# drapado/PINGS

Measured on AMD Instinct MI355X. Metric: raster fwd+bwd Mpix/s @1M Gaussians 1080p, higher is better.
Workload: dtype f32; 1 GPU; surfel rasteriser fwd+bwd, 1000000 Gaussians, 1920x1080, one view per GPU; gaussians=1000000, width=1920, height=1080

## Files before the change

### pings_amd/csrc/raster_blend_fwd.hip

```cpp
#include "raster_common.hpp"

namespace pings {
namespace raster {

template <int MODE>
__device__ __forceinline__ void blend_fwd_wave_body(
    const KParams& p, const uint2* __restrict__ ranges, const uint32_t* __restrict__ point_list,
    const float4* __restrict__ rec, const uint32_t* __restrict__ gval, float* __restrict__ out_color,
    float* __restrict__ out_normal, float* __restrict__ out_depth, float* __restrict__ out_alpha,
    float* __restrict__ final_T, uint32_t* __restrict__ n_contrib, float* __restrict__ inst_wq,
    uint32_t* __restrict__ inst_cntq, const uint32_t* __restrict__ tile_order,
    const uint32_t* __restrict__ seg_tile_unit0, const unsigned block) {
  __shared__ float4 sA_[4][64], sB_[4][64], sC_[4][64], sD_[4][64];
  __shared__ uint32_t sSlot_[4][64];
  __shared__ int sE_[4][64];
  __shared__ float sW_[4][64];
  __shared__ uint32_t sCnt_[4][64];

  const int lane = threadIdx.x & 63, q = (int)(threadIdx.x >> 6);
  float4 *sA = sA_[q], *sB = sB_[q], *sC = sC_[q], *sD = sD_[q];
  uint32_t *sSlot = sSlot_[q], *sCnt = sCnt_[q];
  int* sE = sE_[q];
  float* sW = sW_[q];
  const int tile = (int)tile_order[block];
// ... 714 lines not shown
  for (int k = 0; k < PPL; ++k) {
    if (!inside[k]) continue;
    const int r = k >> 1, h = k & 1;
    const float Tk = T[r][h];
    const size_t pix_id = (size_t)pix_y[r] * p.W + pix_x[h];
    const float A = 1.0f - Tk;
    final_T[pix_id] = Tk;
    n_contrib[pix_id] = last[k];
    out_color[pix_id] = C0[r][h] + Tk * p.bg[0];
    out_color[HW + pix_id] = C1[r][h] + Tk * p.bg[1];
    out_color[2 * HW + pix_id] = C2[r][h] + Tk * p.bg[2];
    out_alpha[pix_id] = A;
    if (MODE == MODE_SURFEL) {
      out_normal[pix_id] = N0[r][h];
      out_normal[HW + pix_id] = N1[r][h];
      out_normal[2 * HW + pix_id] = N2[r][h];
      out_depth[pix_id] = D[r][h] / fmaxf(A, DEPTH_ALPHA_EPS);
    } else {
      out_depth[pix_id] = D[r][h];
    }
  }
  uint32_t mc = 0u;
#pragma unroll
  for (int k = 0; k < PPL; ++k) mc = max(mc, inside[k] ? last[k] : 0u);
#pragma unroll
  for (int off = 32; off > 0; off >>= 1) mc = max(mc, (uint32_t)__shfl_xor((int)mc, off, 64));
  if (lane == 0) tile_maxc[tile] = mc;
}

template <int MODE>
__global__ __launch_bounds__(256) void combine_quadrants_kernel(int64_t I, const float4* __restrict__ wq,
                                                                const uint4* __restrict__ cq, float* __restrict__ inst_w,
                                                                uint32_t* __restrict__ inst_cnt,
                                                                uint8_t* __restrict__ inst_qmask) {
  const int64_t i = (int64_t)blockIdx.x * blockDim.x + threadIdx.x;
  if (i == 0) { inst_w[I] = 0.f; inst_qmask[I] = 0; }
  if (i >= I) return;
  const float4 w = wq[i];
  inst_w[i] = ((w.x + w.y) + w.z) + w.w;
  inst_qmask[i] = (uint8_t)((w.x != 0.f ? 1u : 0u) | (w.y != 0.f ? 2u : 0u) | (w.z != 0.f ? 4u : 0u) | (w.w != 0.f ? 8u : 0u));
  if (MODE == MODE_3DGS) {
    const uint4 c = cq[i];
    inst_cnt[i] = c.x + c.y + c.z + c.w;
  }
}

__device__ inline uint32_t wave_reduce_sum_u32(uint32_t v) {
#pragma unroll
  for (int off = 32; off > 0; off >>= 1) v += (uint32_t)__shfl_xor((int)v, off, 64);
  return v;
}

constexpr int SMALL_RUN = 16;
template <typename T>
__global__ __launch_bounds__(256) void per_gaussian_sum_kernel(
    int P, const uint4* __restrict__ rect, const uint32_t* __restrict__ rank_of,
    const uint32_t* __restrict__ offsets_sorted, const uint32_t* __restrict__ tiles_sorted,
    const T* __restrict__ inst, T* __restrict__ out) {
  const int g = blockIdx.x * blockDim.x + threadIdx.x;
  const int lane = threadIdx.x & 63;
  uint32_t n = 0, base = 0;
  if (g < P && rect[g].w != 0u) {
    const uint32_t r = rank_of[g];
    n = tiles_sorted[r];
    base = offsets_sorted[r] - n;
  }
  T sum = (T)0;
  if (n <= (uint32_t)SMALL_RUN)
    for (uint32_t k = 0; k < n; ++k) sum += inst[base + k];
  unsigned long long m = __ballot(n > (uint32_t)SMALL_RUN);
  while (m) {
    const int src = __ffsll((long long)m) - 1;
    m &= m - 1;
    const uint32_t nb = lane_value(n, src);
    const uint32_t bb = lane_value(base, src);
    T acc = (T)0, acc1 = (T)0, acc2 = (T)0, acc3 = (T)0;
    uint32_t k = lane;
    for (; k + 192 < nb; k += 256) {
      acc += inst[bb + k];
      acc1 += inst[bb + k + 64];
      acc2 += inst[bb + k + 128];
      acc3 += inst[bb + k + 192];
    }
    for (; k < nb; k += 64) acc += inst[bb + k];
    acc = (acc + acc1) + (acc2 + acc3);
    if constexpr (sizeof(T) == 4 && !std::is_integral<T>::value) {
      acc = wave_sum_to_all(acc);
    } else {
      acc = (T)wave_reduce_sum_u32((uint32_t)acc);
    }
    if (lane == src) sum = acc;
  }
  if (g < P) out[g] = sum;
}

struct FwdOut {
  float *color, *normal, *depth, *alpha;
};

template <int MODE>
static int launch_blend_fwd_wave(const KParams& kp, const BlendPlan& plan, int64_t I, int num_tiles, const GeomState& gs,
                          const BinState& bs, const ImageState& im, const FwdOut& o, hipStream_t st) {
  const uint32_t seg = plan.seg;
  if (I > 0) PINGS_HIP_CHECK(hipMemsetAsync(bs.inst_wq, 0, 16 * (size_t)I, st));
  if (I > 0 && MODE == MODE_3DGS) PINGS_HIP_CHECK(hipMemsetAsync(bs.inst_cntq, 0, 16 * (size_t)I, st));
  if (!plan.seg_on) {
    hipLaunchKernelGGL((blend_fwd_wave_kernel<MODE>), dim3(num_tiles), dim3(256), 0, st, kp, bs.ranges,
                       bs.point_list, gs.rec, bs.gval, o.color, o.normal, o.depth, o.alpha,
                       im.final_T, im.n_contrib, bs.inst_wq, bs.inst_cntq, bs.tile_order,
                       (const uint32_t*)nullptr);
  } else {
    hipLaunchKernelGGL(seg_plan_kernel, dim3(1), dim3(1024), 0, st, bs.ranges, num_tiles, 2u * seg, seg,
                       bs.seg_max_units, bs.seg_head, bs.seg_unit_tile, bs.seg_unit_seg, bs.seg_tile_unit0);
    PINGS_LAUNCH_CHECK();
    const dim3 gseg(bs.seg_max_units);
    uint16_t* const rel = plan.seg_reuse ? bs.seg_rel : nullptr;
    uint32_t* const nrel = plan.seg_reuse ? bs.seg_nrel : nullptr;
    hipLaunchKernelGGL((blend_fwd_wave_segT_kernel<MODE>), dim3((unsigned)num_tiles + bs.seg_max_units), dim3(256), 0,
                       st, kp, bs.ranges, bs.point_list, gs.rec, bs.gval, o.color, o.normal, o.depth,
                       o.alpha, im.final_T, im.n_contrib, bs.inst_wq, bs.inst_cntq, bs.tile_order,
                       bs.seg_tile_unit0, (unsigned)num_tiles, seg, bs.seg_head, bs.seg_unit_tile,
                       bs.seg_unit_seg, bs.seg_P, rel, nrel);
    if (plan.seg_reuse)
      hipLaunchKernelGGL((blend_fwd_seg_kernel<MODE, 1, true>), gseg, dim3(256), 0, st, kp, bs.ranges, bs.point_list,
                         gs.rec, bs.gval, seg, bs.seg_head, bs.seg_unit_tile, bs.seg_unit_seg, bs.seg_P, bs.seg_slab,
                         bs.inst_wq, bs.inst_cntq, rel, nrel);
    else
      hipLaunchKernelGGL((blend_fwd_seg_kernel<MODE, 1, false>), gseg, dim3(256), 0, st, kp, bs.ranges, bs.point_list,
                         gs.rec, bs.gval, seg, bs.seg_head, bs.seg_unit_tile, bs.seg_unit_seg, bs.seg_P, bs.seg_slab,
                         bs.inst_wq, bs.inst_cntq, rel, nrel);
    hipLaunchKernelGGL((blend_fwd_seg_combine_kernel<MODE>), gseg, dim3(256), 0, st, kp, bs.ranges, seg, bs.seg_head,
                       bs.seg_unit_tile, bs.seg_unit_seg, bs.seg_slab, o.color, o.normal, o.depth,
                       o.alpha, im.final_T, im.n_contrib);
    PINGS_LAUNCH_CHECK();
  }
  if (I > 0)
    hipLaunchKernelGGL((combine_quadrants_kernel<MODE>), dim3((unsigned)pings::ceil_div<int64_t>(I, 256)),
                       dim3(256), 0, st, I, reinterpret_cast<const float4*>(bs.inst_wq),
                       reinterpret_cast<const uint4*>(bs.inst_cntq), bs.inst_w, bs.inst_cnt, bs.inst_qmask);
  PINGS_LAUNCH_CHECK();
  return PINGS_OK;
}

int launch_blend_fwd(int mode, const KParams& kp, const BlendPlan& plan, int P, int64_t I, const GeomState& gs,
                     const BinState& bs, const ImageState& im, float* out_color, float* out_normal, float* out_depth,
                     float* out_alpha, void* per_gaussian, hipStream_t st) {
  const int num_tiles = kp.gx * kp.gy;
  const FwdOut o{out_color, out_normal, out_depth, out_alpha};
  {
    pings::prof::Scope ps_blend("blend_fwd", st);
    const int e = with_mode(mode, [&](auto m) -> int {
      constexpr int M = m();
      switch (plan.fwd) {
        case BlendPlan::FWD_TILE:
          hipLaunchKernelGGL((blend_fwd_tile_kernel<M>), dim3(num_tiles), dim3(64), 0, st, kp, bs.ranges,
                             bs.point_list, gs.rec, bs.gval, o.color, o.normal, o.depth, o.alpha,
                             im.final_T, im.n_contrib, bs.inst_w, bs.inst_cnt, bs.tile_order, bs.tile_maxc);
          break;
        case BlendPlan::FWD_WAVE:
          if (int e = launch_blend_fwd_wave<M>(kp, plan, I, num_tiles, gs, bs, im, o, st)) return e;
      }
      PINGS_LAUNCH_CHECK();
      return PINGS_OK;
    });
    if (e) return e;
  }
  if (P > 0) {
    pings::prof::Scope ps("per_gaussian_sum", st);
    const dim3 grid(pings::ceil_div(P, 256)), block(256);
    if (I == 0) {
      PINGS_HIP_CHECK(hipMemsetAsync(per_gaussian, 0, 4 * (size_t)P, st));
    } else if (mode == PINGS_RASTER_SURFEL) {
      hipLaunchKernelGGL(per_gaussian_sum_kernel<float>, grid, block, 0, st, P, gs.rect, gs.rank_of,
                         gs.offsets_sorted, gs.tiles_sorted, (const float*)bs.inst_w,
                         reinterpret_cast<float*>(per_gaussian));
    } else {
      hipLaunchKernelGGL(per_gaussian_sum_kernel<uint32_t>, grid, block, 0, st, P, gs.rect, gs.rank_of,
                         gs.offsets_sorted, gs.tiles_sorted, (const uint32_t*)bs.inst_cnt,
                         reinterpret_cast<uint32_t*>(per_gaussian));
    }
    PINGS_LAUNCH_CHECK();
  }
  return PINGS_OK;
}

}
}
```

### pings_amd/csrc/raster_bwd.hip

```cpp
#include <hipcub/hipcub.hpp>

#include <algorithm>
#include <type_traits>

#include "raster_common.hpp"

namespace pings {
namespace raster {

constexpr int BATCH = 64;
constexpr uint32_t LONG_TILES_MAX = 2048;
constexpr uint32_t DEAD_ROW = 0xFFFFFFFFu;

template <int MODE>
__device__ __forceinline__ void blend_bwd_tile_body(
    BParams p, const uint2* __restrict__ ranges, const uint32_t* __restrict__ point_list,
    const float4* __restrict__ rec, const uint32_t* __restrict__ gval, const float* __restrict__ final_T,
    const uint32_t* __restrict__ n_contrib, const float* __restrict__ out_depth, const float* __restrict__ dL_dcolor,
    const float* __restrict__ dL_dnormal, const float* __restrict__ dL_ddepth, const float* __restrict__ dL_dalpha,
    const float* __restrict__ inst_w, const uint32_t* __restrict__ cidx, float* __restrict__ rows,
    const uint32_t* __restrict__ tile_order) {
  __shared__ float4 sA[BATCH], sB[BATCH], sC[BATCH], sD[BATCH];
  __shared__ uint32_t sRow[BATCH];
  __shared__ float4 sG[BATCH][4];
// ... 567 lines not shown
        dst[2] = make_float4(v[8], v[9], v[10], v[11]);
        dst[3] = make_float4(v[12], v[13], v[14], v[15]);
      }
    } else {
      if (gl == lane) {
#pragma unroll
        for (int k = 0; k < 16; ++k) sV[wv][k][lane] = v[k];
      }
      __syncthreads();
      if (act && gl == lane) {
        float o4[4];
#pragma unroll
        for (int u = 0; u < 4; ++u) {
          const int k = 4 * wv + u;
          o4[u] = ((sV[0][k][lane] + sV[1][k][lane]) + sV[2][k][lane]) + sV[3][k][lane];
        }
        dst[wv] = make_float4(o4[0], o4[1], o4[2], o4[3]);
      }
      __syncthreads();
    }
  }
#ifdef PINGS_BWD_STATS
  if (lane == 0) {
    atomicAdd(&g_bwd_stats[0], st_chunks); atomicAdd(&g_bwd_stats[1], st_dead); atomicAdd(&g_bwd_stats[2], st_any);
    atomicAdd(&g_bwd_stats[3], st_exec); atomicAdd(&g_bwd_stats[4], st_valid); atomicAdd(&g_bwd_stats[5], st_take);
  }
#endif
}


__global__ __launch_bounds__(256) void row_chunk_sum_kernel(RowRanges rr, const uint32_t* __restrict__ pair_off,
                                                             const uint32_t* __restrict__ pair_owner,
                                                             const float* __restrict__ rows,
                                                             float* __restrict__ partials) {
  const uint32_t q = (uint32_t)((blockIdx.x * (size_t)blockDim.x + threadIdx.x) >> 4);
  const int c = threadIdx.x & 15;
  if (q >= pair_off[rr.P]) return;
  const uint32_t r = pair_owner[q];
  const uint32_t j = q - pair_off[r];
  const uint32_t row_end = rr.row_end(r);
  uint32_t row = rr.row_begin(r) + j * (uint32_t)CH;
  const uint32_t stop = min(row + (uint32_t)CH, row_end);
  float a0 = 0.f, a1 = 0.f, a2 = 0.f, a3 = 0.f;
  for (; row + 4 <= stop; row += 4) {
    a0 += rows[(size_t)row * 16 + c];
    a1 += rows[(size_t)(row + 1) * 16 + c];
    a2 += rows[(size_t)(row + 2) * 16 + c];
    a3 += rows[(size_t)(row + 3) * 16 + c];
  }
  for (; row < stop; ++row) a0 += rows[(size_t)row * 16 + c];
  partials[(size_t)q * 16 + c] = (a0 + a1) + (a2 + a3);
}

template <int MODE>
__global__ __launch_bounds__(256, 4) void gaussian_bwd_kernel(
    BParams p, const float* __restrict__ means3D, const float* __restrict__ scales,
    const float* __restrict__ rotations, const uint4* __restrict__ rect, const uint32_t* __restrict__ rank_of,
    const uint32_t* __restrict__ tiles_sorted, const uint32_t* __restrict__ pair_off,
    const float* __restrict__ partials, float* __restrict__ dL_dmeans3D, float* __restrict__ dL_dmeans2D, float* __restrict__ dL_dcolors,
    float* __restrict__ dL_dopacities, float* __restrict__ dL_dscales,
    float* __restrict__ dL_drotations, float* __restrict__ tau_partials) {
  __shared__ float sTau[256 / 64][6];
  const int g = blockIdx.x * blockDim.x + threadIdx.x;
  float tau[6] = {0.f, 0.f, 0.f, 0.f, 0.f, 0.f};

  if (g < p.P) {
    uint32_t n_tiles = 0u, qa = 0u, qb = 0u;
    if (rect[g].w != 0u) {
      const uint32_t rank = rank_of[g];
      n_tiles = tiles_sorted[rank];
      qa = pair_off[rank];
      qb = pair_off[rank + 1];
    }
    float G[16];
#pragma unroll
    for (int k = 0; k < 16; ++k) G[k] = 0.f;
    const float4* prow = reinterpret_cast<const float4*>(partials);
    for (uint32_t k = qa; k < qb; ++k) {
#pragma unroll
      for (int q4 = 0; q4 < 4; ++q4) {
        const float4 r = prow[(size_t)k * 4 + q4];
        G[q4 * 4 + 0] += r.x;
        G[q4 * 4 + 1] += r.y;
        G[q4 * 4 + 2] += r.z;
        G[q4 * 4 + 3] += r.w;
      }
    }

    float gm[3] = {0.f, 0.f, 0.f}, gs[3] = {0.f, 0.f, 0.f}, gq4[4] = {0.f, 0.f, 0.f, 0.f};
    float g2d[2] = {0.f, 0.f};
    if (n_tiles > 0 && qb > qa) {
      const float* V = p.view;
      const float* Pm = p.proj_raw;
      const float x = means3D[3 * g], y = means3D[3 * g + 1], z = means3D[3 * g + 2];
      const float px = ((V[0] * x + V[4] * y) + V[8] * z) + V[12];
      const float py = ((V[1] * x + V[5] * y) + V[9] * z) + V[13];
      const float pz = ((V[2] * x + V[6] * y) + V[10] * z) + V[14];
      float gp[3] = {0.f, 0.f, 0.f};
      {
        const float hx = ((Pm[0] * px + Pm[4] * py) + Pm[8] * pz) + Pm[12];
        const float hy = ((Pm[1] * px + Pm[5] * py) + Pm[9] * pz) + Pm[13];
        const float hw = ((Pm[3] * px + Pm[7] * py) + Pm[11] * pz) + Pm[15];
        const float pw = 1.0f / (hw + 1e-7f);
        const float gndx = 0.5f * (float)p.W * G[G_MX];
        const float gndy = 0.5f * (float)p.H * G[G_MY];
        g2d[0] = gndx;
// ... 99 lines not shown
          for (int a = 0; a < 3; ++a) gWc[a][b] += sgn * gn[a] * R[b][2];
        }
        gpz_direct += G[G_ZLO] + G[G_ZHI];
        const float grz = 3.0f * (G[G_ZHI] - G[G_ZLO]);
        if (S[0] > S[1]) gS[0] += grz;
        else if (S[1] > S[0]) gS[1] += grz;
        else { gS[0] += 0.5f * grz; gS[1] += 0.5f * grz; }
      }
      gp[2] += gpz_direct;
      gq4[0] = 2.0f * (-qz * gR[0][1] + qy * gR[0][2] + qz * gR[1][0] - qx * gR[1][2] - qy * gR[2][0] + qx * gR[2][1]);
      gq4[1] = 2.0f * (qy * gR[0][1] + qz * gR[0][2] + qy * gR[1][0] - 2.0f * qx * gR[1][1] - qr * gR[1][2] + qz * gR[2][0] + qr * gR[2][1] - 2.0f * qx * gR[2][2]);
      gq4[2] = 2.0f * (-2.0f * qy * gR[0][0] + qx * gR[0][1] + qr * gR[0][2] + qx * gR[1][0] + qz * gR[1][2] - qr * gR[2][0] + qz * gR[2][1] - 2.0f * qy * gR[2][2]);
      gq4[3] = 2.0f * (-2.0f * qz * gR[0][0] - qr * gR[0][1] + qx * gR[0][2] + qr * gR[1][0] - 2.0f * qz * gR[1][1] + qy * gR[1][2] + qx * gR[2][0] + qy * gR[2][1]);
#pragma unroll
      for (int k = 0; k < 3; ++k) gs[k] = p.scale_mod * gS[k];
#pragma unroll
      for (int b = 0; b < 3; ++b)
        gm[b] = (V[4 * b + 0] * gp[0] + V[4 * b + 1] * gp[1]) + V[4 * b + 2] * gp[2];
      tau[0] = gp[0]; tau[1] = gp[1]; tau[2] = gp[2];
      float th0 = py * gp[2] - pz * gp[1];
      float th1 = pz * gp[0] - px * gp[2];
      float th2 = px * gp[1] - py * gp[0];
#pragma unroll
      for (int b = 0; b < 3; ++b) {
        const float w0 = V[4 * b + 0], w1 = V[4 * b + 1], w2 = V[4 * b + 2];
        th0 += w1 * gWc[2][b] - w2 * gWc[1][b];
        th1 += w2 * gWc[0][b] - w0 * gWc[2][b];
        th2 += w0 * gWc[1][b] - w1 * gWc[0][b];
      }
      tau[3] = th0; tau[4] = th1; tau[5] = th2;
    }
    dL_dmeans3D[3 * g] = gm[0]; dL_dmeans3D[3 * g + 1] = gm[1]; dL_dmeans3D[3 * g + 2] = gm[2];
    dL_dmeans2D[3 * g] = g2d[0]; dL_dmeans2D[3 * g + 1] = g2d[1]; dL_dmeans2D[3 * g + 2] = 0.f;
    dL_dcolors[3 * g] = G[G_R]; dL_dcolors[3 * g + 1] = G[G_G]; dL_dcolors[3 * g + 2] = G[G_B];
    dL_dopacities[g] = G[G_OPAC];
    dL_dscales[3 * g] = gs[0]; dL_dscales[3 * g + 1] = gs[1]; dL_dscales[3 * g + 2] = gs[2];
    dL_drotations[4 * g] = gq4[0]; dL_drotations[4 * g + 1] = gq4[1];
    dL_drotations[4 * g + 2] = gq4[2]; dL_drotations[4 * g + 3] = gq4[3];
  }

  const int lane = threadIdx.x & 63, wave = threadIdx.x >> 6;
#pragma unroll
  for (int k = 0; k < 6; ++k) {
    const float s = wave_reduce_sum_dpp(tau[k]);
    if (lane == 63) sTau[wave][k] = s;
  }
  __syncthreads();
  if (threadIdx.x < 6) {
    const int k = threadIdx.x;
    tau_partials[(size_t)blockIdx.x * 6 + k] = ((sTau[0][k] + sTau[1][k]) + sTau[2][k]) + sTau[3][k];
  }
}

__global__ __launch_bounds__(256) void tau_reduce_kernel(const float* __restrict__ partials, int nblocks,
                                                          float* __restrict__ dL_dtau) {
  __shared__ double sRed[4][6];
  double s[6] = {0, 0, 0, 0, 0, 0};
  for (int i = threadIdx.x; i < nblocks; i += 256) {
#pragma unroll
    for (int k = 0; k < 6; ++k) s[k] += (double)partials[(size_t)i * 6 + k];
  }
#pragma unroll
  for (int k = 0; k < 6; ++k) {
#pragma unroll
    for (int off = 32; off > 0; off >>= 1) s[k] += __shfl_down(s[k], off, 64);
    if ((threadIdx.x & 63) == 0) sRed[threadIdx.x >> 6][k] = s[k];
  }
  __syncthreads();
  if (threadIdx.x < 6)
    dL_dtau[threadIdx.x] = (float)(((sRed[0][threadIdx.x] + sRed[1][threadIdx.x]) + sRed[2][threadIdx.x]) + sRed[3][threadIdx.x]);
}

}
}

using namespace pings::raster;

PINGS_API int pings_raster_backward(const pings_raster_settings* s, int P, int64_t I,
                                    const float* means3D, const float* colors,
                                    const float* opacities, const float* scales,
                                    const float* rotations, const void* geom_blob,
                                    const void* binning_blob, const void* image_blob,
                                    const float* out_color, const float* out_normal,
                                    const float* out_depth, const float* out_alpha,
                                    const float* dL_dcolor, const float* dL_dnormal,
                                    const float* dL_ddepth, const float* dL_dalpha,
                                    void* bwd_blob, float* dL_dmeans3D, float* dL_dmeans2D,
                                    float* dL_dcolors, float* dL_dopacities, float* dL_dscales,
                                    float* dL_drotations, float* dL_dtau, int footprint_class,
                                    void* stream) {
  BParams bp;
  if (int e = fill_camera(s, P, bp)) return e;
  PINGS_ARG_CHECK(dL_dtau != nullptr, "null dL_dtau");
  hipStream_t st = pings::as_stream(stream);
  if (P == 0) {
    PINGS_HIP_CHECK(hipMemsetAsync(dL_dtau, 0, 6 * sizeof(float), st));
    return PINGS_OK;
  }
  PINGS_ARG_CHECK(P > 0 && means3D && colors && opacities && scales && rotations && geom_blob &&
                      binning_blob && image_blob && out_depth && bwd_blob && dL_dmeans3D &&
                      dL_dmeans2D && dL_dcolors && dL_dopacities && dL_dscales && dL_drotations,
                  "null pointer");
  PINGS_ARG_CHECK(I >= 0 && I < (int64_t)0x7FFFFFF0, "instance count out of range");
  (void)out_color; (void)out_normal; (void)out_alpha;
  const RasterKnobs knobs = read_knobs();
  const int num_tiles = bp.gx * bp.gy;
// ... 15 lines not shown
      PINGS_LAUNCH_CHECK();
    }
    order_job.work = fwd_left_it ? bs.tile_maxc : bs.tile_work;
    order_job.num_tiles = num_tiles;
    order_job.order = bs.tile_order + num_tiles;
    order_job.n_long = bs.tile_order + 2 * (size_t)num_tiles;
    order_job.long_thr = plan.long_thr;
    order_job.long_max = LONG_TILES_MAX;
  }
  {
    pings::prof::Scope ps("live_scan", st);
    if (I > 0 && plan.bwd_scan) {
      if (int e = raster_scan_pop(bs.inst_qmask, I + 1, bw.cidx, bw.temp, bw.temp_bytes, knobs.library_scan, order_job, st))
        return e;
    } else if (I > 0) {
      if (int e = raster_scan_live(bs.inst_w, I + 1, bw.cidx, bw.temp, bw.temp_bytes, knobs.library_scan, order_job, st))
        return e;
    } else {
      PINGS_HIP_CHECK(hipMemsetAsync(bw.cidx, 0, 2 * sizeof(uint32_t), st));
    }
    if (int e = raster_scan_chunks(rr, bw.pair_off, bw.pair_owner, bw.temp, bw.temp_bytes, knobs.library_scan, st))
      return e;
  }
  if (I > 0) {
    pings::prof::Scope ps("blend_bwd", st);
    const uint32_t* order = bs.tile_order + num_tiles;
    with_mode(s->mode, [&](auto m) {
      constexpr int M = m();
      if (plan.bwd_scan) {
        const uint32_t* n_long = bs.tile_order + 2 * (size_t)num_tiles;
        const unsigned grid_s = (unsigned)(num_tiles + 3 * std::min<long long>(num_tiles, LONG_TILES_MAX));
        hipLaunchKernelGGL((blend_bwd_scan_kernel<M>), dim3(grid_s), dim3(256), 0, st, bp, bs.ranges,
                           bs.point_list, gs.rec, bs.gval, im.final_T, im.n_contrib, out_depth, dL_dcolor, dL_dnormal,
                           dL_ddepth, dL_dalpha, bs.inst_qmask, bw.cidx, bw.rows, order, n_long);
      } else {
        hipLaunchKernelGGL((blend_bwd_tile_kernel<M>), dim3(num_tiles), dim3(64), 0, st, bp, bs.ranges,
                           bs.point_list, gs.rec, bs.gval, im.final_T, im.n_contrib, out_depth, dL_dcolor,
                           dL_dnormal, dL_ddepth, dL_dalpha, bs.inst_w, bw.cidx, bw.rows, order);
      }
    });
    PINGS_LAUNCH_CHECK();
  }
  {
    pings::prof::Scope ps("row_chunk_sum", st);
    const size_t groups = bw.np_max;
    hipLaunchKernelGGL(row_chunk_sum_kernel, dim3((unsigned)pings::ceil_div<size_t>(groups * 16, 256)),
                       block, 0, st, rr, bw.pair_off, bw.pair_owner, bw.rows, bw.partials);
    PINGS_LAUNCH_CHECK();
  }
  const int nblocks = pings::ceil_div(P, 256);
  {
    pings::prof::Scope ps_g("gaussian_bwd", st);
    with_mode(s->mode, [&](auto m) {
      hipLaunchKernelGGL(gaussian_bwd_kernel<m()>, dim3(nblocks), block, 0, st, bp, means3D,
                         scales, rotations, gs.rect, gs.rank_of, gs.tiles_sorted, bw.pair_off, bw.partials,
                         dL_dmeans3D, dL_dmeans2D, dL_dcolors, dL_dopacities, dL_dscales,
                         dL_drotations, bw.tau_partials);
    });
    PINGS_LAUNCH_CHECK();
    hipLaunchKernelGGL(tau_reduce_kernel, dim3(1), block, 0, st, bw.tau_partials, nblocks, dL_dtau);
    PINGS_LAUNCH_CHECK();
  }
  return PINGS_OK;
}

#ifdef PINGS_BWD_STATS
PINGS_API int pings_debug_bwd_stats(unsigned long long* out8, int reset) {
  PINGS_HIP_CHECK(hipDeviceSynchronize());
  PINGS_HIP_CHECK(hipMemcpyFromSymbol(out8, HIP_SYMBOL(pings::raster::g_bwd_stats), 64));
  if (reset) {
    unsigned long long z[8] = {0};
    PINGS_HIP_CHECK(hipMemcpyToSymbol(HIP_SYMBOL(pings::raster::g_bwd_stats), z, 64));
  }
  return PINGS_OK;
}
#endif
```

### pings_amd/csrc/raster_common.hpp

```cpp
#pragma once
#include <cstdlib>
#include <type_traits>

#include "common.hpp"

namespace pings {
namespace raster {

constexpr int TILE = 16;
constexpr int BLOCK = TILE * TILE;
constexpr float NEAR_Z = 0.2f;
constexpr float LOWPASS = 0.3f;
constexpr float ALPHA_MAX = 0.99f;
constexpr float ALPHA_MIN = 1.0f / 255.0f;
constexpr float T_EPS = 1e-4f;
constexpr float DEPTH_ALPHA_EPS = 1e-10f;
constexpr float DEN_EPS = 1e-6f;
constexpr uint32_t CULLED_KEY = 0xFFFFFFFFu;
constexpr int DS_NB = 1 << 20;
constexpr uint32_t DS_LIMIT = 4096u;
constexpr int DS_SHARDS = 64;
constexpr int DS_KMIN = 2 * DS_SHARDS, DS_SHIFT = DS_KMIN + 1, DS_FLAG = DS_KMIN + 2, DS_HEAD = DS_KMIN + 8;
constexpr float OCC_THR = 9.5f;
constexpr float OCC_FIX = 4096.f;
// ... 106 lines not shown
  const float* view;
  const float* proj_raw;
  const float* bg;
  const float* prcp;
};

template <typename Params>
int fill_camera(const pings_raster_settings* s, int P, Params& kp) {
  PINGS_ARG_CHECK(s != nullptr, "null settings");
  PINGS_ARG_CHECK(s->image_height > 0 && s->image_width > 0, "empty image");
  PINGS_ARG_CHECK(s->image_height < 65536 * TILE / 16 && s->image_width < 65536, "image too large");
  PINGS_ARG_CHECK(s->mode == PINGS_RASTER_SURFEL || s->mode == PINGS_RASTER_3DGS, "unknown mode");
  PINGS_ARG_CHECK(s->viewmatrix && s->projmatrix_raw && s->bg, "null camera pointer");
  PINGS_ARG_CHECK(s->tanfovx > 0 && s->tanfovy > 0, "non-positive tanfov");
  kp.P = P;
  kp.W = s->image_width;
  kp.H = s->image_height;
  kp.gx = ceil_div(kp.W, TILE);
  kp.gy = ceil_div(kp.H, TILE);
  kp.front_only = s->front_only;
  kp.fx = (float)((double)kp.W / (2.0 * s->tanfovx));
  kp.fy = (float)((double)kp.H / (2.0 * s->tanfovy));
  kp.limx = (float)(1.3 * s->tanfovx);
  kp.limy = (float)(1.3 * s->tanfovy);
  kp.scale_mod = (float)s->scale_modifier;
  kp.view = s->viewmatrix;
  kp.proj_raw = s->projmatrix_raw;
  kp.bg = s->bg;
  kp.prcp = s->prcppoint;
  return PINGS_OK;
}

template <typename F>
decltype(auto) with_mode(int mode, F&& f) {
  if (mode == PINGS_RASTER_SURFEL) return f(std::integral_constant<int, MODE_SURFEL>{});
  return f(std::integral_constant<int, MODE_3DGS>{});
}

struct RasterKnobs {
  enum Bwd { BWD_AUTO, BWD_PIXEL, BWD_SCAN };
  int blend_ppl = 0;
  Bwd blend_bwd = BWD_AUTO;
  uint32_t blend_seg = 512u;
  bool seg_reuse = true;
  uint32_t bwd_long = 3072u;
  bool occlusion = true;
  bool library_sort = false;
  bool library_tile_sort = false;
  bool library_scan = false;
  float occ_amin = 0.15f;
  bool occ_walk_lanes = false;
  int rect_rule = RECT_TIGHT;
  bool mark_depth_only = false;
};
RasterKnobs read_knobs();

struct BlendPlan {
  enum Fwd { FWD_TILE, FWD_WAVE } fwd;
  bool want_qmask;
  bool bwd_scan;
  uint32_t seg;
  bool seg_on, seg_reuse;
  uint32_t long_thr;
};
BlendPlan blend_plan(const RasterKnobs& k, int footprint_class, int64_t I, int num_tiles);

struct BwdState {
  uint32_t* cidx;
  float* rows;
  uint32_t *pair_off, *pair_owner;
  float* partials;
  float* tau_partials;
  char* temp;
  size_t temp_bytes, np_max, total;
};

GeomState carve_geom(void* blob, int P, int num_tiles);
int launch_tile_order(const uint32_t* work, int num_tiles, uint32_t* order, hipStream_t st, uint32_t* n_long = nullptr,
                      uint32_t long_thr = 0, uint32_t long_max = 0);
int occlusion_buckets(int num_tiles);
BinState carve_binning(void* blob, int64_t I, int num_tiles, uint32_t seg);
ImageState carve_image(void* blob, int W, int H);
BwdState carve_bwd(void* blob, int P, int64_t I);

constexpr int TS_THREADS = 256, TS_BLOCK = 4096;
size_t tile_sort_table_bytes(int64_t n);
template <typename KeyT>
int tile_sort(const KeyT* keys_in, int64_t n, int bits, KeyT* keys_tmp, uint32_t* vals_tmp, KeyT* keys_out,
              uint32_t* vals_out, uint32_t* table, hipStream_t st);
size_t tile_sort_library_bytes(int64_t n);
template <typename KeyT>
int tile_sort_library(const KeyT* keys_in, int64_t n, int bits, KeyT* keys_out, uint32_t* vals_out, void* temp,
                      size_t temp_bytes, hipStream_t st);

int launch_blend_fwd(int mode, const KParams& kp, const BlendPlan& plan, int P, int64_t I, const GeomState& gs,
                     const BinState& bs, const ImageState& im, float* out_color, float* out_normal, float* out_depth,
                     float* out_alpha, void* per_gaussian, hipStream_t st);

__device__ inline int lane_value(int v, int src) { return __builtin_amdgcn_readlane(v, src); }
__device__ inline uint32_t lane_value(uint32_t v, int src) { return (uint32_t)__builtin_amdgcn_readlane((int)v, src); }
__device__ inline float lane_value(float v, int src) {
  return __builtin_bit_cast(float, __builtin_amdgcn_readlane(__builtin_bit_cast(int, v), src));
}

typedef float f2 __attribute__((ext_vector_type(2)));
__device__ inline f2 f2s(float x) { return f2{x, x}; }
__device__ inline f2 fma2(f2 a, f2 b, f2 c) { return __builtin_elementwise_fma(a, b, c); }
__device__ inline f2 sel2(bool c0, bool c1, f2 a, f2 b) { return f2{c0 ? a.x : b.x, c1 ? a.y : b.y}; }

typedef unsigned long long lmask;
struct cmask {
  unsigned long long bits;
};
enum { LM_OGT = 2, LM_OGE = 3, LM_OLT = 4, LM_OLE = 5 };
__device__ inline cmask mask_lt(float a, float b) { return cmask{__builtin_amdgcn_fcmpf(a, b, LM_OLT)}; }
__device__ inline cmask mask_le(float a, float b) { return cmask{__builtin_amdgcn_fcmpf(a, b, LM_OLE)}; }
// ... 304 lines not shown
```

### pings_amd/csrc/raster_layout.hip

```cpp
#include <hipcub/hipcub.hpp>

#include <algorithm>
#include <cmath>
#include <cstdlib>
#include <cstring>

#include "raster_common.hpp"

namespace pings {
namespace raster {

static size_t sort_temp_bytes(int64_t n) {
  size_t a = 0, b = 0;
  (void)hipcub::DeviceRadixSort::SortPairs(nullptr, a, (uint32_t*)nullptr, (uint32_t*)nullptr,
                                     (uint32_t*)nullptr, (uint32_t*)nullptr, (int)n, 0, 32);
  (void)hipcub::DeviceScan::InclusiveSum(nullptr, b, (uint32_t*)nullptr, (uint32_t*)nullptr,
                                         (int)std::max<int64_t>(n, DS_NB + n / 256 + 2));
  size_t c = 0;
  (void)hipcub::DeviceRadixSort::SortPairs(nullptr, c, (uint16_t*)nullptr, (uint16_t*)nullptr,
                                           (uint32_t*)nullptr, (uint32_t*)nullptr, (int)n, 0, 16);
  if (c > a) a = c;
  a = std::max(a, std::max(tile_sort_library_bytes(n), tile_sort_table_bytes(n)));
  a = std::max(a, raster_scan_bytes(std::max<int64_t>(n, DS_NB + n / 256 + 2)));
  return align_up(a > b ? a : b) + 256;
// ... 72 lines not shown
  const bool reuse = sg > 0 && sg <= 65535;
  b.seg_rel = c.take<uint16_t>(reuse ? (size_t)b.seg_max_units * 4 * sg : 1);
  b.seg_nrel = c.take<uint32_t>((size_t)b.seg_max_units * 4);
  b.temp_bytes = sort_temp_bytes((int64_t)n);
  b.temp = c.take<char>(b.temp_bytes);
  b.total = c.off;
  return b;
}

ImageState carve_image(void* blob, int W, int H) {
  Carver c(blob);
  ImageState im;
  im.final_T = c.take<float>((size_t)W * H);
  im.n_contrib = c.take<uint32_t>((size_t)W * H);
  im.total = c.off;
  return im;
}

BwdState carve_bwd(void* blob, int P, int64_t I) {
  Carver c(blob);
  BwdState b;
  const size_t ni = (size_t)(I > 0 ? I : 1), n = 4 * ni, np = (size_t)(P > 0 ? P : 1);
  b.np_max = n / CH + np + 1;
  b.cidx = c.take<uint32_t>(ni + 2);
  b.pair_off = c.take<uint32_t>(np + 1);
  b.pair_owner = c.take<uint32_t>(b.np_max);
  b.partials = c.take<float>(b.np_max * GRAD_ROW);
  b.tau_partials = c.take<float>((size_t)ceil_div((int)np, 256) * 6);
  b.temp_bytes = std::max(raster_scan_bytes((int64_t)ni + 1), raster_scan_bytes((int64_t)np + 1));
  b.temp = c.take<char>(b.temp_bytes);
  b.rows = c.take<float>(n * GRAD_ROW);
  b.total = c.off;
  return b;
}

RasterKnobs read_knobs() {
  RasterKnobs k;
  if (const char* e = getenv("PINGS_BLEND_PPL")) k.blend_ppl = atoi(e);
  if (const char* e = getenv("PINGS_BLEND_BWD")) k.blend_bwd = strcmp(e, "pixel") != 0 ? RasterKnobs::BWD_SCAN : RasterKnobs::BWD_PIXEL;
  if (const char* e = getenv("PINGS_BLEND_SEG")) k.blend_seg = (uint32_t)atoi(e);
  if (const char* e = getenv("PINGS_BLEND_SEG_REUSE")) k.seg_reuse = atoi(e) != 0;
  if (const char* e = getenv("PINGS_BWD_LONG")) {
    const long v = atol(e);
    k.bwd_long = v <= 0 ? 0xFFFFFFF0u : (uint32_t)((v + 15) / 16 * 16);
  }
  if (const char* e = getenv("PINGS_RASTER_OCCLUSION")) k.occlusion = atoi(e) != 0;
  if (const char* e = getenv("PINGS_DEPTH_SORT")) k.library_sort = e[0] == 'l';
  if (const char* e = getenv("PINGS_TILE_SORT")) k.library_tile_sort = e[0] == 'l';
  if (const char* e = getenv("PINGS_RASTER_SCAN")) k.library_scan = e[0] == 'l';
  if (const char* e = getenv("PINGS_OCC_AMIN")) k.occ_amin = fminf(fmaxf((float)atof(e), 1.0f / 255.0f), 0.99f);
  if (const char* e = getenv("PINGS_OCC_WALK")) k.occ_walk_lanes = e[0] == 'l';
  if (const char* e = getenv("PINGS_RASTER_RECT")) k.rect_rule = e[0] == '3' ? RECT_3SIGMA : e[0] == 'e' ? RECT_ELLIPSE : RECT_TIGHT;
  if (const char* e = getenv("PINGS_MARK_VISIBLE")) k.mark_depth_only = e[0] == 'd';
  return k;
}

BlendPlan blend_plan(const RasterKnobs& k, int footprint_class, int64_t I, int num_tiles) {
  BlendPlan p;
  p.bwd_scan = k.blend_bwd == RasterKnobs::BWD_AUTO ? footprint_class != 2 : k.blend_bwd == RasterKnobs::BWD_SCAN;
  p.want_qmask = p.bwd_scan;
  const bool tile_wave = k.blend_ppl == 4 || (k.blend_ppl == 0 && footprint_class == 2 && !p.want_qmask);
  p.fwd = tile_wave ? BlendPlan::FWD_TILE : BlendPlan::FWD_WAVE;
  p.seg = k.blend_seg;
  p.seg_on = p.seg > 0 && I > (int64_t)num_tiles * (p.seg / 4) && I > 2 * (int64_t)p.seg;
  p.seg_reuse = p.seg <= 65535u && k.seg_reuse;
  p.long_thr = k.bwd_long;
  return p;
}

}
}

using namespace pings::raster;

PINGS_API size_t pings_raster_geom_bytes(int P, int image_height, int image_width) {
  const int nt = pings::ceil_div(image_width, TILE) * pings::ceil_div(image_height, TILE);
  return carve_geom(nullptr, P, nt).total;
}

PINGS_API size_t pings_raster_binning_bytes(int64_t num_instances, int image_height,
                                            int image_width) {
  const int nt = pings::ceil_div(image_width, TILE) * pings::ceil_div(image_height, TILE);
  return carve_binning(nullptr, num_instances, nt, read_knobs().blend_seg).total;
}

PINGS_API size_t pings_raster_backward_bytes(int P, int64_t num_instances) {
  return carve_bwd(nullptr, P, num_instances).total;
}

PINGS_API size_t pings_raster_image_bytes(int image_height, int image_width) {
  return carve_image(nullptr, image_width, image_height).total;
}

__global__ void slots_to_ids_kernel(int64_t I, const uint32_t* __restrict__ list, const uint32_t* __restrict__ gval,
                                    uint32_t* __restrict__ out) {
  const int64_t i = (int64_t)blockIdx.x * blockDim.x + threadIdx.x;
  if (i < I) out[i] = gval[list[i]];
}


PINGS_API int pings_raster_debug_lists(const void* binning_blob, int64_t I, int image_height,
                                       int image_width, uint32_t* point_list, uint32_t* ranges_xy,
                                       void* stream) {
  PINGS_ARG_CHECK(binning_blob && ranges_xy, "null pointer");
  const int nt = pings::ceil_div(image_width, TILE) * pings::ceil_div(image_height, TILE);
  BinState bs = carve_binning(const_cast<void*>(binning_blob), I, nt, read_knobs().blend_seg);
  hipStream_t st = pings::as_stream(stream);
  if (I > 0 && point_list) {
    hipLaunchKernelGGL(slots_to_ids_kernel, dim3((unsigned)pings::ceil_div<int64_t>(I, 256)), dim3(256), 0, st, I,
                       bs.point_list, bs.gval, point_list);
    PINGS_LAUNCH_CHECK();
  }
  PINGS_HIP_CHECK(hipMemcpyAsync(ranges_xy, bs.ranges, sizeof(uint2) * (size_t)nt,
                                 hipMemcpyDeviceToDevice, st));
  return PINGS_OK;
}

PINGS_API int pings_raster_debug_occlusion(const void* geom_blob, int P, int image_height, int image_width,
                                           uint32_t* occ_bucket, uint16_t* occ_bsat, int32_t* occ_nb, void* stream) {
// ... 25 lines not shown
```

Before: 2477 Mpix/s.

## Iterate per-gaussian sum and backward chain over depth-sorted rank order

Adds rank-ordered variants of the per-gaussian instance-sum kernel and the gaussian backward kernel. They walk only the valid sorted Gaussians, either strided across lanes or by chunk owner, and zero-fill culled entries separately. The aim is to skip idle threads for culled Gaussians and read run data from compacted sorted arrays, at the cost of scattered writes through gidx_sorted. The new paths turn on only for particular plan conditions: tile-wave forward for the sum, pixel-based backward for the chain.

```diff
diff --git a/pings_amd/csrc/raster_blend_fwd.hip b/pings_amd/csrc/raster_blend_fwd.hip
--- a/pings_amd/csrc/raster_blend_fwd.hip
+++ b/pings_amd/csrc/raster_blend_fwd.hip
@@ -790,19 +790,9 @@
 }
 
 constexpr int SMALL_RUN = 16;
+
 template <typename T>
-__global__ __launch_bounds__(256) void per_gaussian_sum_kernel(
-    int P, const uint4* __restrict__ rect, const uint32_t* __restrict__ rank_of,
-    const uint32_t* __restrict__ offsets_sorted, const uint32_t* __restrict__ tiles_sorted,
-    const T* __restrict__ inst, T* __restrict__ out) {
-  const int g = blockIdx.x * blockDim.x + threadIdx.x;
-  const int lane = threadIdx.x & 63;
-  uint32_t n = 0, base = 0;
-  if (g < P && rect[g].w != 0u) {
-    const uint32_t r = rank_of[g];
-    n = tiles_sorted[r];
-    base = offsets_sorted[r] - n;
-  }
+__device__ __forceinline__ T wave_run_sums(uint32_t n, uint32_t base, const T* __restrict__ inst, int lane) {
   T sum = (T)0;
   if (n <= (uint32_t)SMALL_RUN)
     for (uint32_t k = 0; k < n; ++k) sum += inst[base + k];
@@ -829,7 +819,51 @@
     }
     if (lane == src) sum = acc;
   }
+  return sum;
+}
+
+template <typename T>
+__global__ __launch_bounds__(256) void per_gaussian_sum_kernel(
+    int P, const uint4* __restrict__ rect, const uint32_t* __restrict__ rank_of,
+    const uint32_t* __restrict__ offsets_sorted, const uint32_t* __restrict__ tiles_sorted,
+    const T* __restrict__ inst, T* __restrict__ out) {
+  const int g = blockIdx.x * blockDim.x + threadIdx.x;
+  const int lane = threadIdx.x & 63;
+  uint32_t n = 0, base = 0;
+  if (g < P && rect[g].w != 0u) {
+    const uint32_t r = rank_of[g];
+    n = tiles_sorted[r];
+    base = offsets_sorted[r] - n;
+  }
+  const T sum = wave_run_sums(n, base, inst, lane);
   if (g < P) out[g] = sum;
+}
+
+template <typename T>
+__global__ __launch_bounds__(256) void per_gaussian_sum_rank_kernel(
+    int P, const uint32_t* __restrict__ depth_key, const uint32_t* __restrict__ rank_of,
+    const uint32_t* __restrict__ gidx_sorted, const uint32_t* __restrict__ offsets_sorted,
+    const uint32_t* __restrict__ tiles_sorted, const uint32_t* __restrict__ nvalid, const T* __restrict__ inst,
+    T* __restrict__ out) {
+  const uint32_t t = blockIdx.x * blockDim.x + threadIdx.x;
+  const int lane = threadIdx.x & 63;
+  if (t < (uint32_t)P) {
+    bool owner = false;
+    if (depth_key[t] != CULLED_KEY) owner = tiles_sorted[rank_of[t]] > 0u;
+    if (!owner) out[t] = (T)0;
+  }
+  const uint32_t nv = *nvalid;
+  const uint32_t nw = (nv + 63u) >> 6, w = t >> 6;
+  if (w >= nw) return;
+  const uint32_t r = (uint32_t)lane * nw + w;
+  uint32_t n = 0, base = 0, g = 0;
+  if (r < nv) {
+    n = tiles_sorted[r];
+    base = offsets_sorted[r] - n;
+    g = gidx_sorted[r];
+  }
+  const T sum = wave_run_sums(n, base, inst, lane);
+  if (n > 0u) out[g] = sum;
 }
 
 struct FwdOut {
@@ -908,6 +942,15 @@
     const dim3 grid(pings::ceil_div(P, 256)), block(256);
     if (I == 0) {
       PINGS_HIP_CHECK(hipMemsetAsync(per_gaussian, 0, 4 * (size_t)P, st));
+    } else if (plan.sum_dense) {
+      if (mode == PINGS_RASTER_SURFEL)
+        hipLaunchKernelGGL(per_gaussian_sum_rank_kernel<float>, grid, block, 0, st, P, gs.depth_key, gs.rank_of,
+                           gs.gidx_sorted, gs.offsets_sorted, gs.tiles_sorted, gs.nvalid, (const float*)bs.inst_w,
+                           reinterpret_cast<float*>(per_gaussian));
+      else
+        hipLaunchKernelGGL(per_gaussian_sum_rank_kernel<uint32_t>, grid, block, 0, st, P, gs.depth_key, gs.rank_of,
+                           gs.gidx_sorted, gs.offsets_sorted, gs.tiles_sorted, gs.nvalid,
+                           (const uint32_t*)bs.inst_cnt, reinterpret_cast<uint32_t*>(per_gaussian));
     } else if (mode == PINGS_RASTER_SURFEL) {
       hipLaunchKernelGGL(per_gaussian_sum_kernel<float>, grid, block, 0, st, P, gs.rect, gs.rank_of,
                          gs.offsets_sorted, gs.tiles_sorted, (const float*)bs.inst_w,
diff --git a/pings_amd/csrc/raster_bwd.hip b/pings_amd/csrc/raster_bwd.hip
--- a/pings_amd/csrc/raster_bwd.hip
+++ b/pings_amd/csrc/raster_bwd.hip
@@ -643,6 +643,209 @@
   partials[(size_t)q * 16 + c] = (a0 + a1) + (a2 + a3);
 }
 
+template <int AHEAD>
+__device__ __forceinline__ void sum_chunk_partials(const float* __restrict__ partials, uint32_t qa, uint32_t qb,
+                                                   float (&G)[16]) {
+#pragma unroll
+  for (int k = 0; k < 16; ++k) G[k] = 0.f;
+  const float4* prow = reinterpret_cast<const float4*>(partials);
+  uint32_t k = qa;
+  if (AHEAD > 1) {
+    for (; k + AHEAD <= qb; k += AHEAD) {
+      float4 r[AHEAD][4];
+#pragma unroll
+      for (int u = 0; u < AHEAD; ++u)
+#pragma unroll
+        for (int q4 = 0; q4 < 4; ++q4) r[u][q4] = prow[(size_t)(k + u) * 4 + q4];
+#pragma unroll
+      for (int u = 0; u < AHEAD; ++u)
+#pragma unroll
+        for (int q4 = 0; q4 < 4; ++q4) {
+          G[q4 * 4 + 0] += r[u][q4].x;
+          G[q4 * 4 + 1] += r[u][q4].y;
+          G[q4 * 4 + 2] += r[u][q4].z;
+          G[q4 * 4 + 3] += r[u][q4].w;
+        }
+    }
+  }
+  for (; k < qb; ++k) {
+#pragma unroll
+    for (int q4 = 0; q4 < 4; ++q4) {
+      const float4 r = prow[(size_t)k * 4 + q4];
+      G[q4 * 4 + 0] += r.x;
+      G[q4 * 4 + 1] += r.y;
+      G[q4 * 4 + 2] += r.z;
+      G[q4 * 4 + 3] += r.w;
+    }
+  }
+}
+
+template <int MODE>
+__device__ inline void gaussian_chain(const BParams& p, int g, const float (&G)[16],
+                                               const float* __restrict__ means3D, const float* __restrict__ scales,
+                                               const float* __restrict__ rotations, float (&gm)[3], float (&gs)[3],
+                                               float (&gq4)[4], float (&g2d)[2], float (&tau)[6]) {
+  const float* V = p.view;
+  const float* Pm = p.proj_raw;
+  const float x = means3D[3 * g], y = means3D[3 * g + 1], z = means3D[3 * g + 2];
+  const float px = ((V[0] * x + V[4] * y) + V[8] * z) + V[12];
+  const float py = ((V[1] * x + V[5] * y) + V[9] * z) + V[13];
+  const float pz = ((V[2] * x + V[6] * y) + V[10] * z) + V[14];
+  float gp[3] = {0.f, 0.f, 0.f};
+  {
+    const float hx = ((Pm[0] * px + Pm[4] * py) + Pm[8] * pz) + Pm[12];
+    const float hy = ((Pm[1] * px + Pm[5] * py) + Pm[9] * pz) + Pm[13];
+    const float hw = ((Pm[3] * px + Pm[7] * py) + Pm[11] * pz) + Pm[15];
+    const float pw = 1.0f / (hw + 1e-7f);
+    const float gndx = 0.5f * (float)p.W * G[G_MX];
+    const float gndy = 0.5f * (float)p.H * G[G_MY];
+    g2d[0] = gndx;
+    g2d[1] = gndy;
+    const float kx = hx * pw * pw, ky = hy * pw * pw;
+#pragma unroll
+    for (int i = 0; i < 3; ++i)
+      gp[i] = gndx * (Pm[4 * i + 0] * pw - kx * Pm[4 * i + 3]) +
+              gndy * (Pm[4 * i + 1] * pw - ky * Pm[4 * i + 3]);
+  }
+  const float qr = rotations[4 * g], qx = rotations[4 * g + 1], qy = rotations[4 * g + 2],
+              qz = rotations[4 * g + 3];
+  float R[3][3];
+  R[0][0] = 1.0f - 2.0f * (qy * qy + qz * qz); R[0][1] = 2.0f * (qx * qy - qr * qz); R[0][2] = 2.0f * (qx * qz + qr * qy);
+  R[1][0] = 2.0f * (qx * qy + qr * qz); R[1][1] = 1.0f - 2.0f * (qx * qx + qz * qz); R[1][2] = 2.0f * (qy * qz - qr * qx);
+  R[2][0] = 2.0f * (qx * qz - qr * qy); R[2][1] = 2.0f * (qy * qz + qr * qx); R[2][2] = 1.0f - 2.0f * (qx * qx + qy * qy);
+  const float S[3] = {p.scale_mod * scales[3 * g], p.scale_mod * scales[3 * g + 1],
+                      p.scale_mod * scales[3 * g + 2]};
+  float RS[3][3], Mc[3][3];
+#pragma unroll
+  for (int i = 0; i < 3; ++i)
+#pragma unroll
+    for (int k = 0; k < 3; ++k) RS[i][k] = R[i][k] * S[k];
+#pragma unroll
+  for (int a = 0; a < 3; ++a)
+#pragma unroll
+    for (int k = 0; k < 3; ++k)
+      Mc[a][k] = (V[a] * RS[0][k] + V[4 + a] * RS[1][k]) + V[8 + a] * RS[2][k];
+  const float txz = px / pz, tyz = py / pz;
+  const bool clx = (txz < -p.limx) || (txz > p.limx), cly = (tyz < -p.limy) || (tyz > p.limy);
+  const float tx = fminf(p.limx, fmaxf(-p.limx, txz)) * pz;
+  const float ty = fminf(p.limy, fmaxf(-p.limy, tyz)) * pz;
+  const float iz = 1.0f / pz, iz2 = iz * iz;
+  const float J00 = p.fx * iz, J02 = -(p.fx * tx) * iz2, J11 = p.fy * iz, J12 = -(p.fy * ty) * iz2;
+  float T0[3], T1[3];
+#pragma unroll
+  for (int k = 0; k < 3; ++k) {
+    T0[k] = J00 * Mc[0][k] + J02 * Mc[2][k];
+    T1[k] = J11 * Mc[1][k] + J12 * Mc[2][k];
+  }
+  const float ca = ((T0[0] * T0[0] + T0[1] * T0[1]) + T0[2] * T0[2]) + LOWPASS;
+  const float cb = (T0[0] * T1[0] + T0[1] * T1[1]) + T0[2] * T1[2];
+  const float cc = ((T1[0] * T1[0] + T1[1] * T1[1]) + T1[2] * T1[2]) + LOWPASS;
+  (void)ca; (void)cb; (void)cc;
+  const float ga = G[G_CONX], gb = G[G_CONY], gc = G[G_CONZ];
+  float gT0[3], gT1[3], gMc[3][3];
+  float gJ00 = 0.f, gJ02 = 0.f, gJ11 = 0.f, gJ12 = 0.f;
+#pragma unroll
+  for (int k = 0; k < 3; ++k) {
+    gT0[k] = 2.0f * ga * T0[k] + gb * T1[k];
+    gT1[k] = 2.0f * gc * T1[k] + gb * T0[k];
+    gJ00 += gT0[k] * Mc[0][k];
+    gJ02 += gT0[k] * Mc[2][k];
+    gJ11 += gT1[k] * Mc[1][k];
+    gJ12 += gT1[k] * Mc[2][k];
+    gMc[0][k] = J00 * gT0[k];
+    gMc[1][k] = J11 * gT1[k];
+    gMc[2][k] = J02 * gT0[k] + J12 * gT1[k];
+  }
+  gp[2] += -p.fx * iz2 * gJ00 - p.fy * iz2 * gJ11;
+  gp[2] += 2.0f * p.fx * tx * iz2 * iz * gJ02 + 2.0f * p.fy * ty * iz2 * iz * gJ12;
+  const float gtx = -p.fx * iz2 * gJ02, gty = -p.fy * iz2 * gJ12;
+  if (clx) gp[2] += gtx * tx * iz; else gp[0] += gtx;
+  if (cly) gp[2] += gty * ty * iz; else gp[1] += gty;
+  float gRS[3][3], gWc[3][3];
+#pragma unroll
+  for (int b = 0; b < 3; ++b)
+#pragma unroll
+    for (int k = 0; k < 3; ++k)
+      gRS[b][k] = (V[4 * b + 0] * gMc[0][k] + V[4 * b + 1] * gMc[1][k]) + V[4 * b + 2] * gMc[2][k];
+#pragma unroll
+  for (int a = 0; a < 3; ++a)
+#pragma unroll
+    for (int b = 0; b < 3; ++b)
+      gWc[a][b] = (gMc[a][0] * RS[b][0] + gMc[a][1] * RS[b][1]) + gMc[a][2] * RS[b][2];
+  float gR[3][3];
+  float gS[3] = {0.f, 0.f, 0.f};
+#pragma unroll
+  for (int i = 0; i < 3; ++i)
+#pragma unroll
+    for (int k = 0; k < 3; ++k) {
+      gS[k] += gRS[i][k] * R[i][k];
+      gR[i][k] = gRS[i][k] * S[k];
+    }
+  float gpz_direct = G[G_PZ];
+  if (MODE == MODE_SURFEL) {
+    float nx = (V[0] * R[0][2] + V[4] * R[1][2]) + V[8] * R[2][2];
+    float ny = (V[1] * R[0][2] + V[5] * R[1][2]) + V[9] * R[2][2];
+    float nz = (V[2] * R[0][2] + V[6] * R[1][2]) + V[10] * R[2][2];
+    const float q = (nx * px + ny * py) + nz * pz;
+    float sgn = 1.0f;
+    if (!p.front_only && q > 0.0f) sgn = -1.0f;
+    nx *= sgn; ny *= sgn; nz *= sgn;
+    const float gq = G[G_Q];
+    const float gn[3] = {G[G_NX] + gq * px, G[G_NY] + gq * py, G[G_NZ] + gq * pz};
+    gp[0] += gq * nx;
+    gp[1] += gq * ny;
+    gp[2] += gq * nz;
+#pragma unroll
+    for (int b = 0; b < 3; ++b) {
+      gR[b][2] += sgn * ((V[4 * b + 0] * gn[0] + V[4 * b + 1] * gn[1]) + V[4 * b + 2] * gn[2]);
+#pragma unroll
+      for (int a = 0; a < 3; ++a) gWc[a][b] += sgn * gn[a] * R[b][2];
+    }
+    gpz_direct += G[G_ZLO] + G[G_ZHI];
+    const float grz = 3.0f * (G[G_ZHI] - G[G_ZLO]);
+    if (S[0] > S[1]) gS[0] += grz;
+    else if (S[1] > S[0]) gS[1] += grz;
+    else { gS[0] += 0.5f * grz; gS[1] += 0.5f * grz; }
+  }
+  gp[2] += gpz_direct;
+  gq4[0] = 2.0f * (-qz * gR[0][1] + qy * gR[0][2] + qz * gR[1][0] - qx * gR[1][2] - qy * gR[2][0] + qx * gR[2][1]);
+  gq4[1] = 2.0f * (qy * gR[0][1] + qz * gR[0][2] + qy * gR[1][0] - 2.0f * qx * gR[1][1] - qr * gR[1][2] + qz * gR[2][0] + qr * gR[2][1] - 2.0f * qx * gR[2][2]);
+  gq4[2] = 2.0f * (-2.0f * qy * gR[0][0] + qx * gR[0][1] + qr * gR[0][2] + qx * gR[1][0] + qz * gR[1][2] - qr * gR[2][0] + qz * gR[2][1] - 2.0f * qy * gR[2][2]);
+  gq4[3] = 2.0f * (-2.0f * qz * gR[0][0] - qr * gR[0][1] + qx * gR[0][2] + qr * gR[1][0] - 2.0f * qz * gR[1][1] + qy * gR[1][2] + qx * gR[2][0] + qy * gR[2][1]);
+#pragma unroll
+  for (int k = 0; k < 3; ++k) gs[k] = p.scale_mod * gS[k];
+#pragma unroll
+  for (int b = 0; b < 3; ++b)
+    gm[b] = (V[4 * b + 0] * gp[0] + V[4 * b + 1] * gp[1]) + V[4 * b + 2] * gp[2];
+  tau[0] = gp[0]; tau[1] = gp[1]; tau[2] = gp[2];
+  float th0 = py * gp[2] - pz * gp[1];
+  float th1 = pz * gp[0] - px * gp[2];
+  float th2 = px * gp[1] - py * gp[0];
+#pragma unroll
+  for (int b = 0; b < 3; ++b) {
+    const float w0 = V[4 * b + 0], w1 = V[4 * b + 1], w2 = V[4 * b + 2];
+    th0 += w1 * gWc[2][b] - w2 * gWc[1][b];
+    th1 += w2 * gWc[0][b] - w0 * gWc[2][b];
+    th2 += w0 * gWc[1][b] - w1 * gWc[0][b];
+  }
+  tau[3] = th0; tau[4] = th1; tau[5] = th2;
+}
+
+__device__ __forceinline__ void block_reduce_tau(const float (&tau)[6], float (&sTau)[256 / 64][6],
+                                                 float* __restrict__ tau_partials) {
+  const int lane = threadIdx.x & 63, wave = threadIdx.x >> 6;
+#pragma unroll
+  for (int k = 0; k < 6; ++k) {
+    const float s = wave_reduce_sum_dpp(tau[k]);
+    if (lane == 63) sTau[wave][k] = s;
+  }
+  __syncthreads();
+  if (threadIdx.x < 6) {
+    const int k = threadIdx.x;
+    tau_partials[(size_t)blockIdx.x * 6 + k] = ((sTau[0][k] + sTau[1][k]) + sTau[2][k]) + sTau[3][k];
+  }
+}
+
 template <int MODE>
 __global__ __launch_bounds__(256, 4) void gaussian_bwd_kernel(
     BParams p, const float* __restrict__ means3D, const float* __restrict__ scales,
@@ -848,6 +1051,64 @@
   }
 }
 
+template <int MODE>
+__global__ __launch_bounds__(256, 4) void gaussian_bwd_chunk_kernel(
+    BParams p, const float* __restrict__ means3D, const float* __restrict__ scales,
+    const float* __restrict__ rotations, const uint32_t* __restrict__ depth_key, const uint32_t* __restrict__ rank_of,
+    const uint32_t* __restrict__ gidx_sorted, const uint32_t* __restrict__ pair_off,
+    const uint32_t* __restrict__ pair_owner, const float* __restrict__ partials, float* __restrict__ dL_dmeans3D,
+    float* __restrict__ dL_dmeans2D, float* __restrict__ dL_dcolors, float* __restrict__ dL_dopacities,
+    float* __restrict__ dL_dscales, float* __restrict__ dL_drotations, float* __restrict__ tau_partials) {
+  __shared__ float sTau[256 / 64][6];
+  const uint32_t t = blockIdx.x * blockDim.x + threadIdx.x;
+  const uint32_t threads = gridDim.x * blockDim.x;
+  const uint32_t P = (uint32_t)p.P;
+  float tau[6] = {0.f, 0.f, 0.f, 0.f, 0.f, 0.f};
+
+  if (t < P) {
+    bool rows = false;
+    if (depth_key[t] != CULLED_KEY) {
+      const uint32_t rank = rank_of[t];
+      rows = pair_off[rank + 1] > pair_off[rank];
+    }
+    if (!rows) {
+      const size_t g = t;
+      dL_dmeans3D[3 * g] = 0.f; dL_dmeans3D[3 * g + 1] = 0.f; dL_dmeans3D[3 * g + 2] = 0.f;
+      dL_dmeans2D[3 * g] = 0.f; dL_dmeans2D[3 * g + 1] = 0.f; dL_dmeans2D[3 * g + 2] = 0.f;
+      dL_dcolors[3 * g] = 0.f; dL_dcolors[3 * g + 1] = 0.f; dL_dcolors[3 * g + 2] = 0.f;
+      dL_dopacities[g] = 0.f;
+      dL_dscales[3 * g] = 0.f; dL_dscales[3 * g + 1] = 0.f; dL_dscales[3 * g + 2] = 0.f;
+      dL_drotations[4 * g] = 0.f; dL_drotations[4 * g + 1] = 0.f;
+      dL_drotations[4 * g + 2] = 0.f; dL_drotations[4 * g + 3] = 0.f;
+    }
+  }
+
+  const uint32_t np = pair_off[P];
+  for (uint32_t q = t; q < np; q += threads) {
+    const uint32_t r = pair_owner[q];
+    const uint32_t qa = pair_off[r];
+    if (qa != q) continue;
+    const uint32_t qb = pair_off[r + 1];
+    const int g = (int)gidx_sorted[r];
+    float G[16];
+    sum_chunk_partials<4>(partials, qa, qb, G);
+    float gm[3] = {0.f, 0.f, 0.f}, gs[3] = {0.f, 0.f, 0.f}, gq4[4] = {0.f, 0.f, 0.f, 0.f};
+    float g2d[2] = {0.f, 0.f};
+    float tg[6];
+    gaussian_chain<MODE>(p, g, G, means3D, scales, rotations, gm, gs, gq4, g2d, tg);
+#pragma unroll
+    for (int k = 0; k < 6; ++k) tau[k] += tg[k];
+    dL_dmeans3D[3 * g] = gm[0]; dL_dmeans3D[3 * g + 1] = gm[1]; dL_dmeans3D[3 * g + 2] = gm[2];
+    dL_dmeans2D[3 * g] = g2d[0]; dL_dmeans2D[3 * g + 1] = g2d[1]; dL_dmeans2D[3 * g + 2] = 0.f;
+    dL_dcolors[3 * g] = G[G_R]; dL_dcolors[3 * g + 1] = G[G_G]; dL_dcolors[3 * g + 2] = G[G_B];
+    dL_dopacities[g] = G[G_OPAC];
+    dL_dscales[3 * g] = gs[0]; dL_dscales[3 * g + 1] = gs[1]; dL_dscales[3 * g + 2] = gs[2];
+    dL_drotations[4 * g] = gq4[0]; dL_drotations[4 * g + 1] = gq4[1];
+    dL_drotations[4 * g + 2] = gq4[2]; dL_drotations[4 * g + 3] = gq4[3];
+  }
+  block_reduce_tau(tau, sTau, tau_partials);
+}
+
 __global__ __launch_bounds__(256) void tau_reduce_kernel(const float* __restrict__ partials, int nblocks,
                                                           float* __restrict__ dL_dtau) {
   __shared__ double sRed[4][6];
@@ -969,10 +1230,16 @@
   {
     pings::prof::Scope ps_g("gaussian_bwd", st);
     with_mode(s->mode, [&](auto m) {
-      hipLaunchKernelGGL(gaussian_bwd_kernel<m()>, dim3(nblocks), block, 0, st, bp, means3D,
-                         scales, rotations, gs.rect, gs.rank_of, gs.tiles_sorted, bw.pair_off, bw.partials,
-                         dL_dmeans3D, dL_dmeans2D, dL_dcolors, dL_dopacities, dL_dscales,
-                         dL_drotations, bw.tau_partials);
+      if (plan.per_gaussian_dense)
+        hipLaunchKernelGGL(gaussian_bwd_chunk_kernel<m()>, dim3(nblocks), block, 0, st, bp, means3D, scales, rotations,
+                           gs.depth_key, gs.rank_of, gs.gidx_sorted, bw.pair_off, bw.pair_owner, bw.partials,
+                           dL_dmeans3D, dL_dmeans2D, dL_dcolors, dL_dopacities, dL_dscales, dL_drotations,
+                           bw.tau_partials);
+      else
+        hipLaunchKernelGGL(gaussian_bwd_kernel<m()>, dim3(nblocks), block, 0, st, bp, means3D,
+                           scales, rotations, gs.rect, gs.rank_of, gs.tiles_sorted, bw.pair_off, bw.partials,
+                           dL_dmeans3D, dL_dmeans2D, dL_dcolors, dL_dopacities, dL_dscales,
+                           dL_drotations, bw.tau_partials);
     });
     PINGS_LAUNCH_CHECK();
     hipLaunchKernelGGL(tau_reduce_kernel, dim3(1), block, 0, st, bw.tau_partials, nblocks, dL_dtau);
diff --git a/pings_amd/csrc/raster_common.hpp b/pings_amd/csrc/raster_common.hpp
--- a/pings_amd/csrc/raster_common.hpp
+++ b/pings_amd/csrc/raster_common.hpp
@@ -182,6 +182,7 @@
   bool occ_walk_lanes = false;
   int rect_rule = RECT_TIGHT;
   bool mark_depth_only = false;
+  bool per_gaussian_index = false;
 };
 RasterKnobs read_knobs();
 
@@ -192,6 +193,7 @@
   uint32_t seg;
   bool seg_on, seg_reuse;
   uint32_t long_thr;
+  bool sum_dense, per_gaussian_dense;
 };
 BlendPlan blend_plan(const RasterKnobs& k, int footprint_class, int64_t I, int num_tiles);
 
diff --git a/pings_amd/csrc/raster_layout.hip b/pings_amd/csrc/raster_layout.hip
--- a/pings_amd/csrc/raster_layout.hip
+++ b/pings_amd/csrc/raster_layout.hip
@@ -148,6 +148,7 @@
   if (const char* e = getenv("PINGS_OCC_WALK")) k.occ_walk_lanes = e[0] == 'l';
   if (const char* e = getenv("PINGS_RASTER_RECT")) k.rect_rule = e[0] == '3' ? RECT_3SIGMA : e[0] == 'e' ? RECT_ELLIPSE : RECT_TIGHT;
   if (const char* e = getenv("PINGS_MARK_VISIBLE")) k.mark_depth_only = e[0] == 'd';
+  if (const char* e = getenv("PINGS_PER_GAUSSIAN")) k.per_gaussian_index = e[0] == 'i';
   return k;
 }
 
@@ -161,6 +162,8 @@
   p.seg_on = p.seg > 0 && I > (int64_t)num_tiles * (p.seg / 4) && I > 2 * (int64_t)p.seg;
   p.seg_reuse = p.seg <= 65535u && k.seg_reuse;
   p.long_thr = k.bwd_long;
+  p.sum_dense = tile_wave && !k.per_gaussian_index;
+  p.per_gaussian_dense = !p.bwd_scan && !k.per_gaussian_index;
   return p;
 }
 
```

Measured after the change: 2526 Mpix/s, median of 5. 2.0% higher.
